# rahul-rwat/ESMStereo

Measured on AMD Instinct MI355X. Metric: stereo pairs/sec at 384×1248 maxdisp=192; EPE vs reference, higher is better.
Workload: dtype f32; 1 GPU; hot path: cost volume -> 3D stems -> 3D hourglass -> regression -> ESM upsampler (models/ESMStereo.py:700-745), ESMStereo-S gwc 384x1248 md192 B1; variant=S, cv=gwc, global_batch=1, height=384, width=1248, maxdisp=192, parallelism=dp1, graph=True

## Files before the change

### esmstereo_amd/csrc/conv_pair2.hip

```cpp
#include "conv_direct.h"

namespace esm {
namespace conv {
namespace {

constexpr int kP2Threads = 256;
constexpr int kHintPairReg = 1 << 29;

__device__ __forceinline__ float regress_px(const float* __restrict__ cp, int D, int sc) {
#pragma clang fp contract(off)
    float acc = 0.f;
    for (int d0 = 0; d0 < D; d0 += 16) {
        float v[16];
#pragma unroll
        for (int k = 0; k < 16; ++k) v[k] = d0 + k < D ? cp[(d0 + k) * sc] : 0.f;
#pragma unroll
        for (int k = 0; k < 16; ++k)
            if (d0 + k < D) acc = acc + v[k] * static_cast<float>(d0 + k);
    }
    return acc;
}

template <int KA, int SA, int KB, int TH>
struct P2Geo {
// ... 89 lines not shown
        const float v = (ok ? p : a.w)[ok ? c : 0];
        vep = ok ? v : ((k & 1) ? 0.f : 1.f);
    }
    if constexpr (REG) {
#pragma unroll
        for (int i = 0; i < PI; ++i) {
            const int e = i * kP2Threads + tid;
            const int q = e % IC, r = (e / IC) % IR, c = e / (IC * IR);
            const int yi = yi0 + r, xi = xi0 + q;
            vi[i] = 0.f;
            if (e < NIN && c == 0 && yi >= 0 && yi < a.Hi && xi >= 0 && xi < a.Wi) {
                const float v = regress_px(sp0 + yi * sh0 + xi, a.src[0].C, sc0);
                vi[i] = v;
                const bool own_y = (bk_.y == 0 || yi >= yb0) && (bk_.y == static_cast<int>(gridDim.y) - 1 || yi < yb0 + TH);
                const bool own_x = (bk_.x == 0 || xi >= xb0) && (bk_.x == static_cast<int>(gridDim.x) - 1 || xi < xb0 + VB);
                if (own_y && own_x) a.out[b * a.ob + yi * a.oh + xi] = v;
            }
        }
    }
    __builtin_amdgcn_sched_barrier(0);
#pragma unroll
    for (int i = 0; i < PI; ++i) {
        const int e = i * kP2Threads + tid;
        if (e < NIN) in[(e / (IC * IR)) * ICS + ((e / IC) % IR) * ICP + e % IC] = vi[i];
    }
#pragma unroll
    for (int i = 0; i < PWA; ++i) {
        const int e = i * kP2Threads + tid;
        if (e < NWA) wa[e] = vwa[i];
    }
#pragma unroll
    for (int i = 0; i < PWB; ++i) wb[i * kP2Threads + tid] = vwb[i];
    if (tid < 64) ep[tid] = vep;
    __syncthreads();

    for (int i = wave; i < NA; i += kP2Threads / 64) {
        floatx4 acc[2] = {floatx4{0.f, 0.f, 0.f, 0.f}, floatx4{0.f, 0.f, 0.f, 0.f}};
        const float* ib = in + kq * ICS + i * SA * ICP + n * SA;
        const float* wp = wa + kq * 16 + n;
        const int kca = (cin + 3) >> 2;
        if constexpr (TA > 1) {
            if (cin == 1) {
                const float* ib0 = in + i * SA * ICP + n * SA;
#pragma unroll
                for (int kc = 0; kc < (TA + 3) / 4; ++kc) {
                    const int t = 4 * kc + kq;
                    const bool tv = t < TA;
                    const int tt = tv ? t : 0;
                    const float bv = ib0[(tt / KA) * ICP + tt % KA];
                    const float av = wa[tt * CINMAX * 16 + n];
                    acc[kc & 1] = __builtin_amdgcn_mfma_f32_16x16x4f32(tv ? av : 0.f, tv ? bv : 0.f, acc[kc & 1], 0, 0, 0);
                }
            } else {
                for (int kc = 0; kc < kca; ++kc) {
#pragma unroll
                    for (int t = 0; t < TA; ++t) {
                        const int ky = t / KA, kx = t % KA;
                        const float bv = ib[4 * kc * ICS + ky * ICP + kx];
                        const float av = wp[(t * CINMAX + 4 * kc) * 16];
                        acc[t & 1] = __builtin_amdgcn_mfma_f32_16x16x4f32(av, bv, acc[t & 1], 0, 0, 0);
                    }
                }
            }
        } else {
            for (int kc = 0; kc < kca; kc += 2) {
                acc[0] = __builtin_amdgcn_mfma_f32_16x16x4f32(wp[4 * kc * 16], ib[4 * kc * ICS], acc[0], 0, 0, 0);
                if (kc + 1 < kca)
                    acc[1] = __builtin_amdgcn_mfma_f32_16x16x4f32(wp[4 * (kc + 1) * 16], ib[4 * (kc + 1) * ICS], acc[1],
                                                                  0, 0, 0);
            }
        }
        const int ya = ya0 + i, xa = xa0 + n;
        const bool inside = ya >= 0 && ya < a.Ho && xa >= 0 && xa < a.Wo;
#pragma unroll
        for (int j = 0; j < 4; ++j) {
            const int co = 4 * kq + j;
            const float v = act_t<ESM_ACT_GELU>((acc[0][j] + acc[1][j]) * ep[co] + ep[16 + co], 0);
            at[co * ACS + i * AR + n] = inside ? v : 0.f;
        }
    }
    __syncthreads();

    for (int t = wave; t < TH; t += kP2Threads / 64) {
        floatx4 acc[2] = {floatx4{0.f, 0.f, 0.f, 0.f}, floatx4{0.f, 0.f, 0.f, 0.f}};
        const float* ab = at + kq * ACS + t * AR + n;
        const float* wp = wb + kq * 16 + n;
#pragma unroll
        for (int kc = 0; kc < 4; ++kc)
#pragma unroll
            for (int tp = 0; tp < TB; ++tp) {
                const int dy = tp / KB, dx = tp % KB;
                const float bv = ab[4 * kc * ACS + dy * AR + dx];
                const float av = wp[(tp * 16 + 4 * kc) * 16];
                acc[tp & 1] = __builtin_amdgcn_mfma_f32_16x16x4f32(av, bv, acc[tp & 1], 0, 0, 0);
            }
        const int yb = yb0 + t, xb = xb0 + n;
        const bool ok = yb < bd.Ho && xb < bd.Wo && n < VB;
        const __amdgpu_buffer_rsrc_t ro = __builtin_amdgcn_make_buffer_rsrc(
            bd.out + b * bd.ob, static_cast<short>(0),
            4 * ((bd.Cout - 1) * static_cast<int>(bd.oc) + (bd.Ho - 1) * static_cast<int>(bd.oh) + bd.Wo), 0x00020000);
#pragma unroll
        for (int j = 0; j < 4; ++j) {
            const int co = 4 * kq + j;
            const float v = act_t<ESM_ACT_GELU>((acc[0][j] + acc[1][j]) * ep[32 + co] + ep[48 + co], 0);
            const unsigned o = (ok && co < bd.Cout) ? 4u * (co * static_cast<int>(bd.oc) + yb * static_cast<int>(bd.oh) + xb)
                                                    : kOOB;
            store_b32(__float_as_uint(v), ro, static_cast<int>(o), 0);
        }
    }
}

template <int KA, int SA, int KB, int TH, int CINMAX, bool REG = false>
int launch_p2(const esm_conv_desc& a, const esm_conv_desc& b, hipStream_t s) {
    using G = P2Geo<KA, SA, KB, TH>;
    const size_t lds = sizeof(float) * (static_cast<size_t>(CINMAX) * G::ICS + KA * KA * CINMAX * 16 + KB * KB * 256 +
                                        16 * G::ACS + 64);
    constexpr int VB = 16 - KB + 1;
    const dim3 grid(ceil_div(b.Wo, VB), ceil_div(b.Ho, TH), a.B);
    if (grid.y > 65535u || grid.z > 65535u) return arg_error("conv pair: grid too large");
    if constexpr (REG) {
        const int pr = b.ph + a.ph, pc = b.pw + a.pw;
        if (pr < 0 || pc < 0 || TH > G::IR - pr || VB > G::IC - pc ||
            (static_cast<int>(grid.y) - 1) * TH - pr + G::IR < a.Hi || (static_cast<int>(grid.x) - 1) * VB - pc + G::IC < a.Wi)
            return arg_error("conv pair: regressed map not covered by the tiles");
    }
    hipLaunchKernelGGL((pair2_kernel<KA, SA, KB, TH, CINMAX, REG>), grid, dim3(kP2Threads), lds, s, a, b);
    return check_launch("conv pair");
}

template <int KA, int SA, int KB>
int launch_p2_k(const esm_conv_desc& a, const esm_conv_desc& b, hipStream_t s) {
    const long long tiles4 = static_cast<long long>(ceil_div(b.Wo, 16 - KB + 1)) * ceil_div(b.Ho, 4) * a.B;
    const int thsel = (b.hint >> 26) & 3;
    const bool small = thsel ? thsel == 1 : tiles4 < 256;
    const bool tall = thsel == 3 && a.Cin <= 16;
    if constexpr (KA == 5 && KB == 3) {
        if (a.hint & kHintPairReg) {
            if (tall) return launch_p2<KA, SA, KB, 8, 4, true>(a, b, s);
            return small ? launch_p2<KA, SA, KB, 2, 4, true>(a, b, s) : launch_p2<KA, SA, KB, 4, 4, true>(a, b, s);
        }
    }
    if (tall) return a.Cin <= 4 ? launch_p2<KA, SA, KB, 8, 4>(a, b, s) : launch_p2<KA, SA, KB, 8, 16>(a, b, s);
    if (a.Cin <= 4) return small ? launch_p2<KA, SA, KB, 2, 4>(a, b, s) : launch_p2<KA, SA, KB, 4, 4>(a, b, s);
    if (a.Cin <= 16) return small ? launch_p2<KA, SA, KB, 2, 16>(a, b, s) : launch_p2<KA, SA, KB, 4, 16>(a, b, s);
    if (a.Cin <= 32) return small ? launch_p2<KA, SA, KB, 2, 32>(a, b, s) : launch_p2<KA, SA, KB, 4, 32>(a, b, s);
    if constexpr (KA == 1) {
        if (a.Cin > 48) return small ? launch_p2<KA, SA, KB, 2, 64>(a, b, s) : launch_p2<KA, SA, KB, 4, 64>(a, b, s);
    }
    return small ? launch_p2<KA, SA, KB, 2, 48>(a, b, s) : launch_p2<KA, SA, KB, 4, 48>(a, b, s);
}

}

bool pair2_ok(const esm_conv_desc& a, const esm_conv_desc& b) {
    const bool a3 = a.kd > 1 || a.Di > 1 || a.Do > 1, b3 = b.kd > 1 || b.Di > 1 || b.Do > 1;
    if (a3 || b3 || a.transposed || b.transposed || a.shuffle > 1 || b.shuffle > 1) return false;
    if (a.Cout != 16 || a.Cin < 1 || a.Cin > (a.kh == 1 ? 64 : 48) || b.Cin != 16 || b.Cout < 1 || b.Cout > 16)
        return false;
    if (!((a.kh == 3 && (a.stride == 1 || a.stride == 2)) || ((a.kh == 1 || a.kh == 5) && a.stride == 1))) return false;
    if (a.ph != a.pw || b.ph != b.pw || b.stride != 1 || (b.kh != 1 && b.kh != 3)) return false;
    if (a.act != ESM_ACT_GELU || b.act != ESM_ACT_GELU) return false;
    if (a.mul || a.res || a.up || a.out2 || a.post_scale != 1.f) return false;
    if (b.mul || b.res || b.up || b.out2 || b.post_scale != 1.f || !b.out) return false;
    if (b.Hi != a.Ho || b.Wi != a.Wo || b.B != a.B) return false;
    if (b.Ho != b.Hi + 2 * b.ph - b.kh + 1 || b.Wo != b.Wi + 2 * b.pw - b.kw + 1) return false;
    if (a.nsrc > 1)
        for (int i = 0; i < a.nsrc; ++i)
            if (a.src[i].C % 4) return false;
    if (a.hint & kHintPairReg) {
        if (a.kh != 5 || b.kh != 3 || a.Cin != 1 || a.nsrc != 1 || a.src[0].C < 1 || !a.out || a.out == b.out)
            return false;
        if (static_cast<long long>(a.src[0].C) * a.src[0].sc >= (1LL << 31) || a.src[0].sh >= (1 << 28)) return false;
    }
    const long long last = (b.Cout - 1) * b.oc + (b.Ho - 1) * b.oh + b.Wo;
    return 4 * last < static_cast<long long>(kOOB) && b.oc < (1 << 28) && b.oh < (1 << 28);
}

int launch_pair2(const esm_conv_desc& a, const esm_conv_desc& b, hipStream_t s) {
    if (!pair2_ok(a, b)) return arg_error("conv pair: unsupported pair");
    if (a.kh == 5) return b.kh == 3 ? launch_p2_k<5, 1, 3>(a, b, s) : launch_p2_k<5, 1, 1>(a, b, s);
    if (a.kh == 1) return b.kh == 3 ? launch_p2_k<1, 1, 3>(a, b, s) : launch_p2_k<1, 1, 1>(a, b, s);
    if (a.stride == 2) return b.kh == 3 ? launch_p2_k<3, 2, 3>(a, b, s) : launch_p2_k<3, 2, 1>(a, b, s);
    return b.kh == 3 ? launch_p2_k<3, 1, 3>(a, b, s) : launch_p2_k<3, 1, 1>(a, b, s);
}

}
}

extern "C" int esm_conv_pair2_f32(const esm_conv_desc* a, const esm_conv_desc* b, void* stream) {
    if (!a || !b) return esm::arg_error("conv pair: null descriptor");
    return esm::conv::launch_pair2(*a, *b, esm::as_stream(stream));
}
```

### esmstereo_amd/engine.py

```python
from __future__ import annotations

import contextlib
import ctypes
import json
import math
import os
import threading
from dataclasses import dataclass
from typing import Dict, List, Optional, Sequence, Tuple

import torch

from . import _lib
from ._lib import (ACT_GELU, ACT_NONE, ACT_RELU, ACT_RELU6, ACT_SIGMOID, ACT_SILU, EsmConfDesc, EsmConvDesc, EsmShuffleConvDesc,
                   EsmShuffleTailDesc, EsmSmixDesc, check, lib)

__all__ = ["Ctx", "PackedConv", "pack_conv", "run_conv", "run_smix", "run_fmnet", "run_shuffle_tail", "pack_shuffle_tail",
           "ACT_NONE", "ACT_GELU", "ACT_SILU", "ACT_RELU", "ACT_SIGMOID", "ACT_RELU6", "run_dwconv", "cached_pack", "run_convt_1x1",
           "convt_1x1_supported", "pack_conv_split", "run_conv_forked",
           "forked_packs", "run_side_partial"]


def _rup(x: int, m: int) -> int:
    return (x + m - 1) // m * m
# ... 479 lines not shown
        raise ValueError("conv: 1..3 sources")
    x0 = srcs[0]
    if x0.dim() != nd + 2:
        raise ValueError(f"conv: expected a {nd + 2}-D input, got shape {tuple(x0.shape)}")
    dev = x0.device
    B = int(x0.shape[0])
    Di, Hi, Wi = _spatial(x0, nd)
    cin = 0
    for i, s in enumerate(srcs):
        require_device(s, "conv input")
        if s.dim() != nd + 2 or int(s.shape[0]) != B or _spatial(s, nd) != (Di, Hi, Wi):
            raise RuntimeError(f"Sizes of tensors must match except in dimension 1 (conv sources "
                               f"{[tuple(t.shape) for t in srcs]})")
        st = s.stride()
        d.src[i].ptr = s.data_ptr()
        d.src[i].C = int(s.shape[1])
        d.src[i].sb, d.src[i].sc = st[0], st[1]
        d.src[i].sd = st[2] if nd == 3 else 0
        d.src[i].sh = st[-2]
        cin += int(s.shape[1])
    if cin != pc.cin:
        raise RuntimeError(f"conv: input has {cin} channels, layer expects {pc.cin}")
    require_on(dev, "conv", *srcs, pc.w, pc.scale, pc.shift, out, mul, res, up, out2, pre)
    d.nsrc = max(1, len(srcs))
    d.B, d.Cin = B, cin
    d.Di, d.Hi, d.Wi = Di, Hi, Wi
    k, s, p = pc.k, pc.stride, pc.pad
    if pc.transposed:
        if (k, s, p) != (4, 2, 1):
            raise ValueError("transposed conv: only k=4 s=2 p=1")
        Do, Ho, Wo = (2 * Di if nd == 3 else 1), 2 * Hi, 2 * Wi
    else:
        Ho, Wo = (Hi + 2 * p - k) // s + 1, (Wi + 2 * p - k) // s + 1
        Do = (Di + 2 * p - k) // s + 1 if nd == 3 else 1
    if min(Do, Ho, Wo) <= 0:
        raise RuntimeError(f"conv: empty output for input extent {(B, cin, Di, Hi, Wi)}")
    d.Do, d.Ho, d.Wo = Do, Ho, Wo
    d.kd = k if nd == 3 else 1
    d.kh = d.kw = k
    d.stride, d.transposed = s, int(pc.transposed)
    d.pd = p if nd == 3 else 0
    d.ph = d.pw = p
    d.Cout, d.cin_pad, d.cout_pad = pc.cout, pc.cin_pad, pc.cout_pad
    d.w = pc.w.data_ptr()
    d.scale = pc.scale.data_ptr() if pc.scale is not None else None
    d.shift = pc.shift.data_ptr() if pc.shift is not None else None
    d.act = pc.act
    r = int(shuffle)
    d.shuffle = r
    if out is None and alloc_out:
        if r > 1:
            if pc.cout % (r * r):
                raise ValueError("pixel shuffle: Cout not divisible by r^2")
            out = ctx.empty(B, pc.cout // (r * r), Ho * r, Wo * r)
        else:
            out = ctx.empty(B, pc.cout, Do, Ho, Wo) if nd == 3 else ctx.empty(B, pc.cout, Ho, Wo)
    if out is not None:
        require_device(out, "conv output")
        require_on(dev, "conv output", out)
        ost = out.stride()
        d.out = out.data_ptr()
        d.ob, d.oc = ost[0], ost[1]
        d.od = ost[2] if nd == 3 else 0
        d.oh = ost[-2]
    if mul is not None:
        require_device(mul, "conv mul")
        d.mul = mul.data_ptr()
        d.mb, d.mc, d.mh = mul.stride(0), mul.stride(1), mul.stride(-2)
    if res is not None:
        require_device(res, "conv residual")
        if out is None or tuple(res.shape) != tuple(out.shape):
            raise ValueError("conv: residual shape must match the output")
        rs = res.stride()
        d.res = res.data_ptr()
        d.rb, d.rc = rs[0], rs[1]
        d.rd = rs[2] if nd == 3 else 0
        d.rh = rs[-2]
    if up is not None:
        require_device(up, "conv bilinear source")
        d.up = up.data_ptr()
        d.up_h, d.up_w, d.up_f = int(up.shape[-2]), int(up.shape[-1]), int(up_f)
        d.ub, d.uh = up.stride(0), up.stride(-2)
        if d.up_h * up_f != Ho or d.up_w * up_f != Wo:
            raise ValueError("conv: bilinear source extent x factor must equal the output extent")
    d.post_scale = float(post_scale)
    if out2 is not None:
        require_device(out2, "conv out2")
        if out2.stride() != out.stride() or out2.shape != out.shape:
            raise ValueError("conv: out2 must have the output's shape and strides")
        d.out2 = out2.data_ptr()
        d.post_scale2 = float(post_scale2)
    if pre is not None:
        require_device(pre, "conv pre")
        if nd != 2 or pc.transposed or shuffle > 1 or up is not None or tuple(pre.shape) != (B, pc.cout, Ho, Wo):
            raise ValueError("conv: a partial sum (pre) is [B, Cout, Ho, Wo] of a 2-D, non-transposed conv")
        d.pre = pre.data_ptr()
        d.prb, d.prc, d.prh = pre.stride(0), pre.stride(1), pre.stride(2)
    key = conv_key(d, nd)
    d.hint = int(hint) if hint else HINT_SET.get(tag, TUNED_HINTS.get(key, 0))
    if (B * max(Di * Hi * Wi, Do * Ho * Wo) >= XCD_SLAB_MIN_PIX and (nd == 2 or XCD_SLAB_3D)) or \
            (nd == 3 and XCD_SLAB_3D and pc.cin >= 32 and B * Do * Ho * Wo >= XCD_SLAB_MIN_VOX_WIDE) or \
            tag in XCD_SLAB_OPS:
        d.hint |= HINT_XCD_SLAB
    ctx.hold(pc.w, pc.scale, pc.shift, *srcs, out, out2, mul, res, up, pre)
    taps = pc.k ** nd
    if pc.transposed:
        macs = B * Di * Hi * Wi * pc.cin * pc.cout * taps
    else:
        macs = B * Do * Ho * Wo * pc.cin * pc.cout * taps
    in_bytes = 4 * B * cin * Di * Hi * Wi
    out_bytes = 4 * B * pc.cout * Do * Ho * Wo * (2 if out2 is not None else 1)
    extra = 4 * sum(t.numel() for t in (res, mul, up, pre) if t is not None)
    w_bytes = 4 * pc.cin * pc.cout * taps
    meta = dict(name=tag, kind="conv", flops=2 * macs, bytes=in_bytes + out_bytes + extra + w_bytes,
                shape=f"{'T' if pc.transposed else ''}{nd}d k{pc.k}s{pc.stride} {cin}->{pc.cout} "
                      f"in {Di}x{Hi}x{Wi} out {Do}x{Ho}x{Wo}",
                reads=_spans(*srcs, mul, res, up, pre), writes=_spans(out, out2), key=key, hint=d.hint)
    return d, out, meta


GWC_STEM_ENABLED = _ab("ESM_GWC_STEM", "1") != "0"
GWC_STEM_WLDS = _ab("ESM_GWC_STEM_WLDS", "0") == "1"


def gwc_stem_supported(pc: PackedConv, L: torch.Tensor, G: int, D: int, att) -> bool:
    if att is not None or pc.nd != 3 or pc.transposed or (pc.k, pc.stride, pc.pad) != (3, 1, 1):
        return False
    B, C, H, W = (int(v) for v in L.shape)
    if pc.cin != G or G % 4 or C != 2 * G or pc.cout > 8 or not L.is_contiguous():
        return False
    return B * D * H * W >= (1 << 16) and 4 * C * H * W < (1 << 30) and 4 * pc.cout * D * H * W < (1 << 30)


def run_gwc_stem(ctx: Ctx, pc: PackedConv, L: torch.Tensor, R: torch.Tensor, G: int, D: int,
                 tag: str = "gwc_volume+group_stem", hint: int = 0) -> torch.Tensor:
    B, C, H, W = (int(v) for v in L.shape)
    if tuple(R.shape) != (B, C, H, W) or not R.is_contiguous() or not L.is_contiguous():
        raise ValueError("gwc_stem: L and R must be contiguous tensors of one shape")
    virt = L.as_strided((B, G, D, H, W), (0, 0, 0, 0, 1))
    d, out, meta = _conv_desc(ctx, pc, [virt], tag=tag, hint=hint)
    d.hint &= HINT_XCD_SLAB | (3 << 26) | ((1 << 28) if hint else 0)
    if GWC_STEM_WLDS:
        d.hint |= 1 << 28
    vol_flops = 2 * B * C * D * H * W
    meta.update(kind="gwc_stem", flops=meta["flops"] + vol_flops,
                bytes=4 * B * 2 * C * H * W + 4 * B * pc.cout * D * H * W + 4 * pc.cin * pc.cout * 27,
                reads=_spans(L, R), shape=f"gwc G{G} D{D} + " + meta["shape"])
    ctx.meta.append(meta)
    ctx.gwc_stem(d, L, R, C, G)
    return out


PAIR2_ENABLED = _ab("ESM_PAIR2", "1") != "0"


def pair2_supported(pa: PackedConv, pb: PackedConv, srcs: Sequence[torch.Tensor]) -> bool:
    if not PAIR2_ENABLED or pa.nd != 2 or pb.nd != 2 or pa.transposed or pb.transposed:
        return False
    if pa.cout != 16 or pb.cin != 16 or pb.cout > 16 or pa.cin > (64 if pa.k == 1 else 48):
        return False
    if not ((pa.k == 3 and pa.stride in (1, 2)) or (pa.k in (1, 5) and pa.stride == 1)):
        return False
    if pb.stride != 1 or pb.k not in (1, 3) or pa.act != ACT_GELU or pb.act != ACT_GELU:
        return False
    return len(srcs) == 1 or all(int(t.shape[1]) % 4 == 0 for t in srcs)


def pair2_auto(pa: PackedConv, pb: PackedConv, srcs: Sequence[torch.Tensor]) -> bool:
    if not pair2_supported(pa, pb, srcs):
        return False
    B = int(srcs[0].shape[0])
    Ho = (int(srcs[0].shape[2]) + 2 * pa.pad - pa.k) // pa.stride + 1
    Wo = (int(srcs[0].shape[3]) + 2 * pa.pad - pa.k) // pa.stride + 1
    light = pa.cin * pa.k * pa.k
    return pb.k == 1 or (light <= 25 and pa.stride == 1) or (pa.k == 1 and B * Ho * Wo <= 8192)


CONVT1X1_ENABLED = _ab("ESM_CONVT_1X1", "1") != "0"
CONVT1X1_PAIRED = _ab("ESM_CONVT_1X1_PAIRED", "1") == "1"
CONVT1X1_MAX_EXTRA = 48

FORK_ENABLED = _ab("ESM_FORK", "0") == "1"


def convt_1x1_supported(pa: PackedConv, pb: PackedConv, extra: Sequence[torch.Tensor]) -> bool:
    if not CONVT1X1_ENABLED or not pa.transposed or pb.transposed or (pa.k, pa.stride, pa.pad) != (4, 2, 1):
        return False
    wide = pa.cout > 16 or pb.cout > 16
    if pa.act != ACT_GELU or pa.scale is None or pa.shift is None or pa.cout > 32 or pa.cout % 4:
        return False
    if (pb.k, pb.stride, pb.pad) != (1, 1, 0) or pb.act != ACT_GELU or pb.cout > 32 or pb.nd != pa.nd:
        return False
    if wide and (pa.nd != 3 or pa.cout < 2):
        return False
    cx = sum(int(t.shape[1]) for t in extra)
    return 1 <= len(extra) <= 2 and all(int(t.shape[1]) % 4 == 0 for t in extra) and \
        4 <= cx <= (32 if wide else CONVT1X1_MAX_EXTRA)


def run_convt_1x1(ctx: Ctx, pa: PackedConv, srcs: Sequence[torch.Tensor], pb: PackedConv, extra: Sequence[torch.Tensor],
                  tags: Tuple[str, str] = ("convT", "conv1x1"), pre: Optional[torch.Tensor] = None) -> torch.Tensor:
    da, _, ma = _conv_desc(ctx, pa, srcs, tag=tags[0], alloc_out=False)
    nd = pa.nd
    e0 = extra[0]
    geo = (int(e0.shape[0]), pa.cout) + tuple(int(v) for v in e0.shape[2:])
    virt = srcs[0].as_strided(geo, (0,) * (len(geo) - 1) + (1,))
    db, out, mb = _conv_desc(ctx, pb, [virt, *extra], tag=tags[1], pre=pre)
    db.hint = 0
    B = int(e0.shape[0])
    vox = math.prod(int(v) for v in e0.shape[2:])
    full = 4 * B * pa.cout * int(da.Ho) * int(da.Wo) * (int(da.Do) if nd == 3 else 1)
    name = f"{tags[0]}+{'.'.join(tags[1].split('.')[-2:])}"
    ctx.meta.append(dict(name=name, kind="conv_up1", flops=ma["flops"] + mb["flops"],
                         bytes=ma["bytes"] - full + mb["bytes"] - 4 * B * pa.cout * vox,
                         shape=f"{ma['shape']} + {mb['shape']}", reads=ma["reads"] + _spans(*extra), writes=mb["writes"],
                         key=ma["key"] + " | " + mb["key"], hint=da.hint))
    if ctx._submit():
        if ctx.plan:
            ctx._placed(check(lib.esm_plan_add_convt_1x1(ctx.plan, ctypes.byref(da), ctypes.byref(db)), "plan_add_convt_1x1"))
        else:
            check(lib.esm_convt_1x1_f32(ctypes.byref(da), ctypes.byref(db), ctx.stream), "convt_1x1")
    return out


def forked_packs(owner: torch.nn.Module, conv: torch.nn.Module, bn: Optional[torch.nn.Module], act: int, cm: int,
                 cs: int) -> Tuple[PackedConv, PackedConv]:
    def build():
        return (pack_conv_split(conv, None, act, cm, cm + cs), pack_conv_split(conv, bn, act, 0, cm))
    return cached_pack(owner, f"fork{cm}", [conv, bn], build)


def run_side_partial(ctx: Ctx, p_side: PackedConv, side: torch.Tensor, tag: str, cm: int) -> torch.Tensor:
    with ctx.side():
        part = run_conv(ctx, p_side, [side], tag=tag + "[side]")
    ctx.meta[-1].update(layer=tag, split=(cm, cm + p_side.cin))
    ctx.join_next()
    return part


def run_conv_forked(ctx: Ctx, owner: torch.nn.Module, conv: torch.nn.Module, bn: Optional[torch.nn.Module], act: int,
                    main: Sequence[torch.Tensor], side: torch.Tensor, tag: str = "conv") -> torch.Tensor:
    cm = sum(int(t.shape[1]) for t in main)
    p_side, p_main = forked_packs(owner, conv, bn, act, cm, int(side.shape[1]))
    part = run_side_partial(ctx, p_side, side, tag, cm)
    out = run_conv(ctx, p_main, list(main), pre=part, tag=tag)
    ctx.meta[-1].update(layer=tag, split=(0, cm))
    return out


PAIR_REGRESS_ENABLED = _ab("ESM_PAIR_REGRESS", "1") != "0"
PAIR2_TH = {sel: tuple(x for x in _ab(f"ESM_PAIR2_TH{n}", "").split(",") if x)
            for sel, n in ((1, 2), (2, 4), (3, 8))}
HINT_PAIR_REGRESS = 1 << 29


def run_pair2(ctx: Ctx, pa: PackedConv, srcs: Sequence[torch.Tensor], pb: PackedConv,
              tags: Tuple[str, str] = ("convA", "convB"), force: bool = False,
              regress: Optional[torch.Tensor] = None) -> torch.Tensor:
    take = pair2_supported(pa, pb, srcs) if force else pair2_auto(pa, pb, srcs)
    if regress is not None:
        B_, D_, H_, W_ = (int(v) for v in regress.shape)
        init = srcs[0]
        fuse = (take and PAIR_REGRESS_ENABLED and len(srcs) == 1 and pa.k == 5 and pb.k == 3 and pa.cin == 1
                and regress.stride(3) == 1 and tuple(init.shape) == (B_, 1, H_, W_) and init.stride(3) == 1)
        if not fuse:
            ctx.regression(0, regress, init, B_, D_, H_, W_)
            regress = None
    if not take:
        return run_conv(ctx, pb, [run_conv(ctx, pa, srcs, tag=tags[0])], tag=tags[1])
    da, _, ma = _conv_desc(ctx, pa, srcs, tag=tags[0], alloc_out=False)
    da.hint &= ~HINT_PAIR_REGRESS
    B = int(srcs[0].shape[0])
    geo = (B, pa.cout) + ((int(da.Do),) if pa.nd == 3 else ()) + (int(da.Ho), int(da.Wo))
    virt = srcs[0].as_strided(geo, (0,) * (len(geo) - 1) + (1,))
    db, out, mb = _conv_desc(ctx, pb, [virt], tag=tags[1])
    db.hint &= ~(3 << 26)
    for sel, subs in PAIR2_TH.items():
        if any(x in tags[0] for x in subs):
            db.hint |= sel << 26
    mid = 4 * B * pa.cout * int(da.Ho) * int(da.Wo) * (int(da.Do) if pa.nd == 3 else 1)
    name = f"{tags[0]}+{tags[1].rsplit('.', 1)[-1]}"
    flops, byts, reads, writes = ma["flops"] + mb["flops"], ma["bytes"] - mid + mb["bytes"] - mid, ma["reads"], mb["writes"]
    if regress is not None:
        require_on(init.device, "pair regression", regress)
        st = regress.stride()
        da.src[0].ptr, da.src[0].C = regress.data_ptr(), D_
        da.src[0].sb, da.src[0].sc, da.src[0].sh = st[0], st[1], st[2]
        da.out = init.data_ptr()
        da.ob, da.oc, da.oh = init.stride(0), init.stride(1), init.stride(2)
        da.hint |= HINT_PAIR_REGRESS
        ctx.hold(regress, init)
        name = "disparity_regression+" + name
        flops += 2 * B_ * D_ * H_ * W_
        byts += 4 * B_ * D_ * H_ * W_
        reads, writes = _spans(regress), writes + _spans(init)
    ctx.meta.append(dict(name=name, kind="conv_pair", flops=flops, bytes=byts, shape=f"pair {ma['shape']} + {mb['shape']}",
                         reads=reads, writes=writes, key=ma["key"] + " | " + mb["key"], hint=0))
    ctx.pair2(da, db)
    return out


def run_dwconv(ctx: Ctx, x: torch.Tensor, w: torch.Tensor, scale: Optional[torch.Tensor], shift: Optional[torch.Tensor],
               k: int, stride: int, pad: int, act: int, tag: str = "dwconv") -> torch.Tensor:
    if stride <= 0 or k <= 0 or not 0 <= pad < k:
        raise ValueError("dwconv: stride and K must be positive, 0 <= pad < K")
    if x.dim() != 4 or x.stride(3) != 1:
        raise ValueError("dwconv: a [B, C, H, W] input with unit W stride")
    require_device(x, "dwconv input")
    B, C, H, W = (int(v) for v in x.shape)
    Ho, Wo = (H + 2 * pad - k) // stride + 1, (W + 2 * pad - k) // stride + 1
    out = ctx.empty(B, C, Ho, Wo)
    require_on(x.device, "dwconv", x, w, scale, shift, out)
    d = _lib.EsmDwconvDesc()
    d.x, d.xb, d.xc, d.xh = x.data_ptr(), x.stride(0), x.stride(1), x.stride(2)
    d.w = w.data_ptr()
    d.scale = scale.data_ptr() if scale is not None else None
    d.shift = shift.data_ptr() if shift is not None else None
    d.out, d.ob, d.oc, d.oh = out.data_ptr(), out.stride(0), out.stride(1), out.stride(2)
    d.B, d.C, d.H, d.W, d.K, d.stride, d.pad, d.act, d.Ho, d.Wo = B, C, H, W, k, stride, pad, act, Ho, Wo
    ctx.meta.append(dict(name=tag, kind="dwconv", flops=2 * B * C * Ho * Wo * k * k,
                         bytes=4 * (x.numel() + out.numel() + C * k * k), reads=_spans(x), writes=_spans(out)))
    ctx.dwconv(d)
    return out


@dataclass
class SmixStage:
    ln_w: torch.Tensor
    fc0_w: torch.Tensor
    fc0_b: torch.Tensor
    fc2_w: torch.Tensor
    fc2_b: torch.Tensor


def run_smix(ctx: Ctx, x: torch.Tensor, stages: Sequence[SmixStage], *, dw: Optional[Tuple[torch.Tensor, torch.Tensor]] = None,
             res: Optional[torch.Tensor] = None, out: Optional[torch.Tensor] = None, tag: str = "smix") -> torch.Tensor:
    require_device(x, "smix input")
    if not x.is_contiguous():
        raise ValueError("smix: input must be contiguous")
    B, C, H, W = (int(v) for v in x.shape)
    if out is None:
        out = ctx.empty(B, C, H, W)
    d = EsmSmixDesc()
    d.x, d.out = x.data_ptr(), out.data_ptr()
    if res is not None:
        require_device(res, "smix residual")
        if not res.is_contiguous() or res.shape != x.shape:
            raise ValueError("smix: residual must be contiguous and shaped like the input")
        d.res = res.data_ptr()
    if dw is not None:
        d.dw_w, d.dw_b = dw[0].data_ptr(), dw[1].data_ptr()
        d.dw_k = int(dw[0].shape[-1])
    if len(stages) > _lib.SMIX_MAX_STAGES:
        raise ValueError("smix: at most 2 stages per launch")
    require_on(x.device, "smix", x, out, res, *(dw or ()),
               *[t for st in stages for t in (st.ln_w, st.fc0_w, st.fc0_b, st.fc2_w, st.fc2_b)])
    d.nstages = len(stages)
    for i, st in enumerate(stages):
        d.stage[i].ln_w = st.ln_w.data_ptr()
        d.stage[i].fc0_w, d.stage[i].fc0_b = st.fc0_w.data_ptr(), st.fc0_b.data_ptr()
        d.stage[i].fc2_w, d.stage[i].fc2_b = st.fc2_w.data_ptr(), st.fc2_b.data_ptr()
        ctx.hold(st.ln_w, st.fc0_w, st.fc0_b, st.fc2_w, st.fc2_b)
    d.B, d.C, d.H, d.W = B, C, H, W
    ctx.hold(x, out, res, *(dw or ()))
    npix = B * H * W
    ctx.meta.append(dict(name=tag, kind="smix", flops=npix * (2 * C * C * len(stages) + (2 * C * d.dw_k ** 2 if dw else 0)),
                         bytes=4 * npix * C * (3 if res is not None else 2), shape=f"C{C} {H}x{W} dw{d.dw_k}",
                         reads=_spans(x, res), writes=_spans(out)))
    ctx.smix(d)
    return out


FM2_MIN_PIX = int(_ab("ESM_FM2_MIN_PIX", "16384"))


def run_fmnet(ctx: Ctx, x: torch.Tensor, stages: Sequence[SmixStage], dw0: Tuple[torch.Tensor, torch.Tensor],
              dw1: Tuple[torch.Tensor, torch.Tensor], out: Optional[torch.Tensor] = None,
              tag: str = "fmnet", conv: Optional[Tuple[torch.Tensor, ...]] = None,
              two_launch: Optional[bool] = None) -> torch.Tensor:
    require_device(x, "fmnet input")
    if not x.is_contiguous():
        raise ValueError("fmnet: input must be contiguous")
    if len(stages) != 4:
        raise ValueError("fmnet: four mlp stages")
    B, C, H, W = (int(v) for v in x.shape)
    if out is None:
        out = ctx.empty(B, C, H, W)
    d = _lib.EsmFmnetDesc()
    d.x, d.out = x.data_ptr(), out.data_ptr()
    d.dw_w[0], d.dw_b[0] = dw0[0].data_ptr(), dw0[1].data_ptr()
    d.dw_w[1], d.dw_b[1] = dw1[0].data_ptr(), dw1[1].data_ptr()
    d.dw_k = int(dw0[0].shape[-1])
    if int(dw1[0].shape[-1]) != d.dw_k:
        raise ValueError("fmnet: both SMLayers need the same depthwise kernel")
    require_on(x.device, "fmnet", x, out, *dw0, *dw1,
               *[t for st in stages for t in (st.ln_w, st.fc0_w, st.fc0_b, st.fc2_w, st.fc2_b)])
    for i, st in enumerate(stages):
        d.stage[i].ln_w = st.ln_w.data_ptr()
        d.stage[i].fc0_w, d.stage[i].fc0_b = st.fc0_w.data_ptr(), st.fc0_b.data_ptr()
        d.stage[i].fc2_w, d.stage[i].fc2_b = st.fc2_w.data_ptr(), st.fc2_b.data_ptr()
        ctx.hold(st.ln_w, st.fc0_w, st.fc0_b, st.fc2_w, st.fc2_b)
    d.B, d.C, d.H, d.W = B, C, H, W
    if conv is not None:
        w0, b0, w2, b2 = conv
        hid = int(w0.shape[0])
        if tuple(w0.shape) != (hid, C, 3, 3) or tuple(w2.shape[:2]) != (C, hid) or hid != C + 16:
            raise ValueError("fmnet: FMBlock.conv must be Conv2d(C, C+16, 3) and Conv2d(C+16, C, 1)")
        for t in conv:
            if not t.is_contiguous():
                raise ValueError("fmnet: conv weights must be contiguous")
        require_on(x.device, "fmnet conv", *conv)
        d.conv0_w, d.conv0_b, d.conv2_w, d.conv2_b = (t.data_ptr() for t in conv)
        d.hid = hid
        ctx.hold(*conv)
        if two_launch is None:
            two_launch = B * H * W >= FM2_MIN_PIX
        if two_launch:
            work = ctx.empty(B, C, H, W)
            d.work = work.data_ptr()
            ctx.hold(work)
    ctx.hold(x, out, *dw0, *dw1)
    npix = B * H * W
    flops = 2 * C * C * 4 + 2 * 2 * C * d.dw_k ** 2 + (2 * d.hid * C * 9 + 2 * C * d.hid if conv is not None else 0)
    ctx.meta.append(dict(name=tag, kind="fmnet", flops=npix * flops,
                         bytes=4 * npix * C * 2 + 4 * (sum(int(t.numel()) for t in conv) if conv is not None else 0),
                         shape=f"C{C} {H}x{W} dw{d.dw_k} x2" + (f" +conv{d.hid}" if conv is not None else ""),
                         reads=_spans(x), writes=_spans(out), launches=2 if d.work else 1))
    ctx.fmnet(d)
    return out
# ... 167 lines not shown
```

Before: 3250 pairs/s.

## Add K-split MFMA fused conv pair kernel for small 3x3 conv pairs

```diff
diff --git a/esmstereo_amd/csrc/conv_pair2.hip b/esmstereo_amd/csrc/conv_pair2.hip
--- a/esmstereo_amd/csrc/conv_pair2.hip
+++ b/esmstereo_amd/csrc/conv_pair2.hip
@@ -265,7 +265,7 @@
 
 }
 
-bool pair2_ok(const esm_conv_desc& a, const esm_conv_desc& b) {
+bool pair2_lds_ok(const esm_conv_desc& a, const esm_conv_desc& b) {
     const bool a3 = a.kd > 1 || a.Di > 1 || a.Do > 1, b3 = b.kd > 1 || b.Di > 1 || b.Do > 1;
     if (a3 || b3 || a.transposed || b.transposed || a.shuffle > 1 || b.shuffle > 1) return false;
     if (a.Cout != 16 || a.Cin < 1 || a.Cin > (a.kh == 1 ? 64 : 48) || b.Cin != 16 || b.Cout < 1 || b.Cout > 16)
@@ -289,8 +289,21 @@
     return 4 * last < static_cast<long long>(kOOB) && b.oc < (1 << 28) && b.oh < (1 << 28);
 }
 
+bool pairk_ok(const esm_conv_desc& a, const esm_conv_desc& b);
+int launch_pairk(const esm_conv_desc& a, const esm_conv_desc& b, hipStream_t s);
+
+constexpr int kHintPairK = 1 << 28;
+
+bool pair2_ok(const esm_conv_desc& a, const esm_conv_desc& b) {
+    if (a.pre || b.pre) return false;
+    return pair2_lds_ok(a, b) || pairk_ok(a, b);
+}
+
 int launch_pair2(const esm_conv_desc& a, const esm_conv_desc& b, hipStream_t s) {
-    if (!pair2_ok(a, b)) return arg_error("conv pair: unsupported pair");
+    if (a.pre || b.pre) return arg_error("conv pair: a partial sum (pre) is not supported on either conv");
+    const bool lds = pair2_lds_ok(a, b);
+    if (((b.hint & kHintPairK) || !lds) && !(a.hint & kHintPairReg) && pairk_ok(a, b)) return launch_pairk(a, b, s);
+    if (!lds) return arg_error("conv pair: unsupported pair");
     if (a.kh == 5) return b.kh == 3 ? launch_p2_k<5, 1, 3>(a, b, s) : launch_p2_k<5, 1, 1>(a, b, s);
     if (a.kh == 1) return b.kh == 3 ? launch_p2_k<1, 1, 3>(a, b, s) : launch_p2_k<1, 1, 1>(a, b, s);
     if (a.stride == 2) return b.kh == 3 ? launch_p2_k<3, 2, 3>(a, b, s) : launch_p2_k<3, 2, 1>(a, b, s);
diff --git a/esmstereo_amd/csrc/conv_pairk.hip b/esmstereo_amd/csrc/conv_pairk.hip
--- /dev/null
+++ b/esmstereo_amd/csrc/conv_pairk.hip
@@ -0,0 +1,313 @@
+#include <algorithm>
+
+#include "conv_direct.h"
+
+namespace esm {
+namespace conv {
+namespace {
+
+constexpr int kPkAR = 18;
+constexpr int kPkVB = 14;
+constexpr size_t kPkMaxLds = 64 * 1024;
+constexpr int kPkWaves = 16;
+
+__device__ __forceinline__ int pk_div(int n, unsigned m) {
+    return m ? static_cast<int>(__umulhi(static_cast<unsigned>(n), m)) : n;
+}
+
+inline unsigned pk_magic(int d) {
+    return d <= 1 ? 0u : static_cast<unsigned>(((1ull << 32) + static_cast<unsigned long long>(d) - 1) / d);
+}
+
+inline int pk_acs(int np, int na) {
+    const int s = np * na * kPkAR;
+    return s + ((16 - s % 32) + 32) % 32;
+}
+
+struct PkGeo {
+    int th;
+    int acs;
+    int red;
+    unsigned m_ga, m_gb, m_do;
+    unsigned m_ca, m_cb;
+};
+
+template <int MT>
+__device__ __forceinline__ void pk_load_wb(float (&av)[9][MT], __amdgpu_buffer_rsrc_t wrs, unsigned wl, int wtap,
+                                           int cout_pad, int g, int dz) {
+#pragma unroll
+    for (int t = 0; t < 9; ++t)
+#pragma unroll
+        for (int mt = 0; mt < MT; ++mt)
+            av[t][mt] = buf_load_s(wrs, wl, 4 * ((dz * 9 + t) * wtap + 4 * g * cout_pad + 16 * mt));
+}
+
+template <bool D3, int SA, int MT, int NW>
+__global__ void __launch_bounds__(64 * NW) pairk_kernel(const esm_conv_desc a, const esm_conv_desc bd, const PkGeo geo) {
+    constexpr int NP = D3 ? 3 : 1;
+    constexpr int KDT = D3 ? 3 : 1;
+    constexpr int TAPS = KDT * 9;
+    extern __shared__ __attribute__((aligned(16))) float lds[];
+    float* red = lds;
+    float* at = red + geo.red;
+    const int TH = geo.th, NA = TH + 2, ACS = geo.acs;
+    const int GA = (a.Cin + 3) >> 2, GB = (bd.Cin + 3) >> 2;
+    const int CPA = 4 * ((a.Cout + 3) >> 2), CPB = 4 * ((bd.Cout + 3) >> 2);
+    float* ep = at + CPA * ACS;
+
+    const int tid = static_cast<int>(threadIdx.x);
+    const int lane = tid & 63, wave = __builtin_amdgcn_readfirstlane(tid >> 6);
+    const int n16 = lane & 15, kq = lane >> 4;
+    const Blk3 bk_ = xcd_block((a.hint & kHintXcd) != 0);
+    const int xb0 = bk_.x * kPkVB, yb0 = bk_.y * TH;
+    const int b = pk_div(bk_.z, geo.m_do);
+    const int zb = bk_.z - b * bd.Do;
+
+    if (tid < 128) {
+        const int k = tid >> 5, c = tid & 31;
+        const float* p = k == 0 ? a.scale : (k == 1 ? a.shift : (k == 2 ? bd.scale : bd.shift));
+        const int cn = k < 2 ? a.Cout : bd.Cout;
+        const bool ok = p != nullptr && c < cn;
+        const float v = (ok ? p : a.w)[ok ? c : 0];
+        ep[tid] = ok ? v : ((k & 1) ? 0.f : 1.f);
+    }
+
+    const int plo = D3 ? max(0, 1 - zb) : 0, phi = D3 ? min(3, a.Do + 1 - zb) : 1;
+    const int ilo = max(0, 1 - yb0), ihi = min(NA, a.Ho + 1 - yb0);
+    const int nvr = ihi - ilo;
+    const int ntask = (phi - plo) * nvr * GA;
+
+    const int xa = xb0 - 1 + n16;
+    unsigned xoff[3];
+#pragma unroll
+    for (int t = 0; t < 3; ++t) {
+        const int xi = xa * SA - a.pw + t;
+        xoff[t] = (xa >= 0 && xa < a.Wo && xi >= 0 && xi < a.Wi) ? 4u * xi : kOOB;
+    }
+    const int wtap = a.cin_pad * a.cout_pad;
+    const __amdgpu_buffer_rsrc_t wrs =
+        __builtin_amdgcn_make_buffer_rsrc(const_cast<float*>(a.w), static_cast<short>(0), 4 * TAPS * wtap, 0x00020000);
+    const unsigned wl = 4u * (kq * a.cout_pad + n16);
+    const int ns = a.nsrc;
+    const int lo1 = a.src[0].C, lo2 = lo1 + (ns > 1 ? a.src[1].C : 0);
+
+    for (int t = wave; t < ntask; t += NW) {
+        const int seg = pk_div(t, geo.m_ga);
+        const int g = t - seg * GA;
+        const int pp = (seg >= nvr ? 1 : 0) + (seg >= 2 * nvr ? 1 : 0);
+        const int za = zb - 1 + plo + pp, ya = yb0 - 1 + ilo + (seg - pp * nvr);
+        const int c0 = 4 * g;
+        const int s = (ns > 1 && c0 >= lo1) ? ((ns > 2 && c0 >= lo2) ? 2 : 1) : 0;
+        const int lo = s == 0 ? 0 : (s == 1 ? lo1 : lo2);
+        const float* sp = s == 0 ? a.src[0].ptr : (s == 1 ? a.src[1].ptr : a.src[2].ptr);
+        const int sC = s == 0 ? a.src[0].C : (s == 1 ? a.src[1].C : a.src[2].C);
+        const long long sb = s == 0 ? a.src[0].sb : (s == 1 ? a.src[1].sb : a.src[2].sb);
+        const int sc = static_cast<int>(s == 0 ? a.src[0].sc : (s == 1 ? a.src[1].sc : a.src[2].sc));
+        const int sd = static_cast<int>(s == 0 ? a.src[0].sd : (s == 1 ? a.src[1].sd : a.src[2].sd));
+        const int sh = static_cast<int>(s == 0 ? a.src[0].sh : (s == 1 ? a.src[1].sh : a.src[2].sh));
+        const int span = 4 * ((sC - 1) * sc + (D3 ? (a.Di - 1) * sd : 0) + (a.Hi - 1) * sh + a.Wi);
+        const __amdgpu_buffer_rsrc_t rs =
+            __builtin_amdgcn_make_buffer_rsrc(const_cast<float*>(sp + b * sb), static_cast<short>(0), span, 0x00020000);
+        const int cl = c0 - lo + kq;
+        const unsigned chv = (c0 + kq < a.Cin && cl < sC) ? 4u * cl * sc : kOOB;
+
+        float bv[TAPS], av[TAPS][MT];
+#pragma unroll
+        for (int dz = 0; dz < KDT; ++dz) {
+            const int zi = D3 ? za * SA - a.pd + dz : 0;
+            const bool zok = !D3 || (zi >= 0 && zi < a.Di);
+#pragma unroll
+            for (int dy = 0; dy < 3; ++dy) {
+                const int yi = ya * SA - a.ph + dy;
+                const int roff = (zok && yi >= 0 && yi < a.Hi) ? 4 * ((D3 ? zi * sd : 0) + yi * sh) : static_cast<int>(kOOB);
+#pragma unroll
+                for (int dx = 0; dx < 3; ++dx) {
+                    const int tap = (dz * 3 + dy) * 3 + dx;
+                    bv[tap] = buf_load_s(rs, chv + xoff[dx], roff);
+#pragma unroll
+                    for (int mt = 0; mt < MT; ++mt)
+                        av[tap][mt] = buf_load_s(wrs, wl, 4 * (tap * wtap + c0 * a.cout_pad + 16 * mt));
+                }
+            }
+        }
+        __builtin_amdgcn_sched_barrier(0);
+        floatx4 acc[2][MT];
+#pragma unroll
+        for (int c = 0; c < 2; ++c)
+#pragma unroll
+            for (int mt = 0; mt < MT; ++mt) acc[c][mt] = floatx4{0.f, 0.f, 0.f, 0.f};
+#pragma unroll
+        for (int tap = 0; tap < TAPS; ++tap)
+#pragma unroll
+            for (int mt = 0; mt < MT; ++mt)
+                acc[tap & 1][mt] = __builtin_amdgcn_mfma_f32_16x16x4f32(av[tap][mt], bv[tap], acc[tap & 1][mt], 0, 0, 0);
+        float* rp = red + t * CPA * 16 + n16;
+#pragma unroll
+        for (int mt = 0; mt < MT; ++mt)
+#pragma unroll
+            for (int j = 0; j < 4; ++j) {
+                const int co = 16 * mt + 4 * kq + j;
+                if (co < CPA) rp[co * 16] = acc[0][mt][j] + acc[1][mt][j];
+            }
+    }
+
+    const int NPB = D3 ? 3 : 1;
+    const int ntb = TH * GB * NPB;
+    const int wtapb = bd.cin_pad * bd.cout_pad;
+    const __amdgpu_buffer_rsrc_t wrsb =
+        __builtin_amdgcn_make_buffer_rsrc(const_cast<float*>(bd.w), static_cast<short>(0), 4 * TAPS * wtapb, 0x00020000);
+    const unsigned wlb = 4u * (kq * bd.cout_pad + n16);
+    float avb[9][MT];
+    {
+        const int tg = pk_div(wave, D3 ? 0x55555556u : 0u);
+        const int dz = wave - tg * NPB;
+        const int g = tg - pk_div(tg, geo.m_gb) * GB;
+        if (wave < ntb) pk_load_wb<MT>(avb, wrsb, wlb, wtapb, bd.cout_pad, g, dz);
+    }
+    __syncthreads();
+
+    {
+        const int nel = NP * NA * CPA * 16;
+        for (int e = tid; e < nel; e += 64 * NW) {
+            const int sgi = pk_div(e, geo.m_ca);
+            const int r = e - sgi * CPA * 16;
+            const int co = r >> 4, n = r & 15;
+            const int p = D3 ? (sgi >= NA ? 1 : 0) + (sgi >= 2 * NA ? 1 : 0) : 0;
+            const int i = sgi - p * NA;
+            const int xc = xb0 - 1 + n;
+            const bool ok = p >= plo && p < phi && i >= ilo && i < ihi && xc >= 0 && xc < a.Wo && co < a.Cout;
+            float v = 0.f;
+            if (ok) {
+                const float* rp = red + ((p - plo) * nvr + (i - ilo)) * GA * CPA * 16 + r;
+                v = rp[0];
+                for (int g = 1; g < GA; ++g) v = v + rp[g * CPA * 16];
+                v = gelu_erf(v * ep[co] + ep[32 + co]);
+            }
+            at[co * ACS + sgi * kPkAR + n] = v;
+        }
+    }
+    __syncthreads();
+
+    for (int tb = wave; tb < ntb; tb += NW) {
+        const int tg = pk_div(tb, D3 ? 0x55555556u : 0u);
+        const int dz = tb - tg * NPB;
+        const int tr = pk_div(tg, geo.m_gb);
+        const int g = tg - tr * GB;
+        if (tb != wave) pk_load_wb<MT>(avb, wrsb, wlb, wtapb, bd.cout_pad, g, dz);
+        const float* ab = at + (4 * g + kq) * ACS + (dz * NA + tr) * kPkAR + n16;
+        float bvb[9];
+#pragma unroll
+        for (int t = 0; t < 9; ++t) bvb[t] = ab[(t / 3) * kPkAR + t % 3];
+        __builtin_amdgcn_sched_barrier(0);
+        floatx4 acc[2][MT];
+#pragma unroll
+        for (int c = 0; c < 2; ++c)
+#pragma unroll
+            for (int mt = 0; mt < MT; ++mt) acc[c][mt] = floatx4{0.f, 0.f, 0.f, 0.f};
+#pragma unroll
+        for (int t = 0; t < 9; ++t)
+#pragma unroll
+            for (int mt = 0; mt < MT; ++mt)
+                acc[t & 1][mt] = __builtin_amdgcn_mfma_f32_16x16x4f32(avb[t][mt], bvb[t], acc[t & 1][mt], 0, 0, 0);
+        float* rp = red + tb * CPB * 16 + n16;
+#pragma unroll
+        for (int mt = 0; mt < MT; ++mt)
+#pragma unroll
+            for (int j = 0; j < 4; ++j) {
+                const int co = 16 * mt + 4 * kq + j;
+                if (co < CPB) rp[co * 16] = acc[0][mt][j] + acc[1][mt][j];
+            }
+    }
+    __syncthreads();
+
+    {
+        const __amdgpu_buffer_rsrc_t ro = __builtin_amdgcn_make_buffer_rsrc(
+            bd.out + b * bd.ob, static_cast<short>(0),
+            4 * ((bd.Cout - 1) * static_cast<int>(bd.oc) + (D3 ? (bd.Do - 1) * static_cast<int>(bd.od) : 0) +
+                 (bd.Ho - 1) * static_cast<int>(bd.oh) + bd.Wo),
+            0x00020000);
+        const int nel = TH * CPB * 16;
+        const int per = GB * NPB;
+        for (int e = tid; e < nel; e += 64 * NW) {
+            const int tr = pk_div(e, geo.m_cb);
+            const int r = e - tr * CPB * 16;
+            const int co = r >> 4, n = r & 15;
+            const float* rp = red + tr * per * CPB * 16 + r;
+            float v = rp[0];
+            for (int k = 1; k < per; ++k) v = v + rp[k * CPB * 16];
+            v = gelu_erf(v * ep[64 + co] + ep[96 + co]);
+            const int yb = yb0 + tr, xb = xb0 + n;
+            const bool ok = n < kPkVB && xb < bd.Wo && yb < bd.Ho && co < bd.Cout;
+            const unsigned vo = ok ? 4u * (co * static_cast<int>(bd.oc) + xb) : kOOB;
+            const int so = 4 * ((D3 ? zb * static_cast<int>(bd.od) : 0) + min(yb, bd.Ho - 1) * static_cast<int>(bd.oh));
+            store_b32(__float_as_uint(v), ro, static_cast<int>(vo), so);
+        }
+    }
+}
+
+size_t pk_geo(const esm_conv_desc& a, const esm_conv_desc& b, bool d3, int th, PkGeo* geo) {
+    const int np = d3 ? 3 : 1, na = th + 2;
+    const int ga = (a.Cin + 3) / 4, gb = (b.Cin + 3) / 4;
+    const int cpa = 4 * ((a.Cout + 3) / 4), cpb = 4 * ((b.Cout + 3) / 4);
+    const int segs = std::min(np, a.Do) * std::min(na, a.Ho);
+    const int red = std::max(segs * ga * cpa * 16, th * gb * np * cpb * 16);
+    const int acs = pk_acs(np, na);
+    if (geo) *geo = PkGeo{th, acs, red, pk_magic(ga), pk_magic(gb), pk_magic(b.Do), pk_magic(cpa * 16), pk_magic(cpb * 16)};
+    return sizeof(float) * (static_cast<size_t>(red) + static_cast<size_t>(cpa) * acs + 128);
+}
+
+template <bool D3, int SA, int MT>
+int launch_pk(const esm_conv_desc& a, const esm_conv_desc& b, hipStream_t s) {
+    const int tiles_w = ceil_div(b.Wo, kPkVB);
+    const long long planes = static_cast<long long>(b.Do) * a.B;
+    const int sel = (b.hint >> 26) & 3;
+    int th = sel == 3 ? 4 : sel;
+    if (!th) {
+        th = 1;
+        while (th < 4 && tiles_w * static_cast<long long>(ceil_div(b.Ho, th)) * planes > 256) th *= 2;
+    }
+    while (th > 1 && pk_geo(a, b, D3, th, nullptr) > kPkMaxLds) th /= 2;
+    PkGeo geo;
+    const size_t lds = pk_geo(a, b, D3, th, &geo);
+    if (lds > kPkMaxLds) return arg_error("conv pair (K-split): tile does not fit LDS");
+    const dim3 grid(tiles_w, ceil_div(b.Ho, th), static_cast<unsigned>(planes));
+    if (grid.y > 65535u || planes > 65535) return arg_error("conv pair (K-split): grid too large");
+    hipLaunchKernelGGL((pairk_kernel<D3, SA, MT, kPkWaves>), grid, dim3(64 * kPkWaves), lds, s, a, b, geo);
+    return check_launch("conv pair (K-split)");
+}
+
+}
+
+bool pairk_ok(const esm_conv_desc& a, const esm_conv_desc& b) {
+    const bool a3 = a.kd > 1 || a.Di > 1 || a.Do > 1, b3 = b.kd > 1 || b.Di > 1 || b.Do > 1;
+    if (a3 != b3 || a.transposed || b.transposed || a.shuffle > 1 || b.shuffle > 1) return false;
+    if (a.kh != 3 || a.kw != 3 || b.kh != 3 || b.kw != 3 || a.kd != (a3 ? 3 : 1) || b.kd != (a3 ? 3 : 1)) return false;
+    if ((a.stride != 1 && a.stride != 2) || b.stride != 1) return false;
+    if (a.ph != 1 || a.pw != 1 || b.ph != 1 || b.pw != 1 || (a3 && (a.pd != 1 || b.pd != 1))) return false;
+    if (a.Cin < 1 || a.Cin > 48 || a.Cout < 1 || a.Cout > 32 || b.Cin != a.Cout || b.Cout < 1 || b.Cout > 32) return false;
+    if (a.act != ESM_ACT_GELU || b.act != ESM_ACT_GELU) return false;
+    if (a.mul || a.res || a.up || a.out2 || a.post_scale != 1.f || a.pre) return false;
+    if (b.mul || b.res || b.up || b.out2 || b.post_scale != 1.f || b.pre || !b.out) return false;
+    if (a.nsrc < 1 || a.nsrc > ESM_MAX_SRC || !direct_ok(a)) return false;
+    int cs = 0;
+    for (int i = 0; i < a.nsrc; ++i) cs += a.src[i].C;
+    if (cs < a.Cin) return false;
+    if (b.B != a.B || b.Di != a.Do || b.Hi != a.Ho || b.Wi != a.Wo || b.Do != b.Di || b.Ho != b.Hi || b.Wo != b.Wi) return false;
+    if (a.Do < 1 || a.Ho < 1 || a.Wo < 1 || a.B < 1) return false;
+    const long long last = (b.Cout - 1) * b.oc + (a3 ? (b.Do - 1) * b.od : 0) + (b.Ho - 1) * b.oh + b.Wo;
+    if (4 * last >= static_cast<long long>(kOOB) || b.oc >= (1 << 28) || b.od >= (1 << 28) || b.oh >= (1 << 28)) return false;
+    return pk_geo(a, b, a3, 1, nullptr) <= kPkMaxLds;
+}
+
+int launch_pairk(const esm_conv_desc& a, const esm_conv_desc& b, hipStream_t s) {
+    if (!pairk_ok(a, b)) return arg_error("conv pair (K-split): unsupported pair");
+    const bool d3 = a.kd > 1;
+    const bool mt2 = a.Cout > 16 || b.Cout > 16;
+#define ESM_PK(D, S) (mt2 ? launch_pk<D, S, 2>(a, b, s) : launch_pk<D, S, 1>(a, b, s))
+    if (d3) return a.stride == 2 ? ESM_PK(true, 2) : ESM_PK(true, 1);
+    return a.stride == 2 ? ESM_PK(false, 2) : ESM_PK(false, 1);
+#undef ESM_PK
+}
+
+}
+}
diff --git a/esmstereo_amd/engine.py b/esmstereo_amd/engine.py
--- a/esmstereo_amd/engine.py
+++ b/esmstereo_amd/engine.py
@@ -655,22 +655,66 @@
 
 
 PAIR2_ENABLED = _ab("ESM_PAIR2", "1") != "0"
+PAIRK_ENABLED = _ab("ESM_PAIRK", "1") != "0"
+PAIRK_MAX_VOX = int(_ab("ESM_PAIRK_MAX_VOX", "4096"))
+HINT_PAIRK = 1 << 28
+
+
+def _pair_out(pa: PackedConv, srcs: Sequence[torch.Tensor]) -> Tuple[int, ...]:
+    ext = tuple((int(v) + 2 * pa.pad - pa.k) // pa.stride + 1 for v in srcs[0].shape[2:])
+    return ((1,) + ext) if pa.nd == 2 else ext
+
+
+def _pair2_lds_supported(pa: PackedConv, pb: PackedConv, srcs: Sequence[torch.Tensor]) -> bool:
+    if pa.nd != 2 or pb.nd != 2 or pa.transposed or pb.transposed:
+        return False
+    if pa.cout != 16 or pb.cin != 16 or pb.cout > 16 or pa.cin > (64 if pa.k == 1 else 48):
+        return False
+    if not ((pa.k == 3 and pa.stride in (1, 2)) or (pa.k in (1, 5) and pa.stride == 1)):
+        return False
+    if pb.stride != 1 or pb.k not in (1, 3) or pa.act != ACT_GELU or pb.act != ACT_GELU:
+        return False
+    return len(srcs) == 1 or all(int(t.shape[1]) % 4 == 0 for t in srcs)
+
+
+def pairk_supported(pa: PackedConv, pb: PackedConv, srcs: Sequence[torch.Tensor]) -> bool:
+    if not PAIR2_ENABLED or pa.nd != pb.nd or pa.transposed or pb.transposed:
+        return False
+    if (pa.k, pa.pad) != (3, 1) or (pb.k, pb.pad, pb.stride) != (3, 1, 1) or pa.stride not in (1, 2):
+        return False
+    if not (1 <= pa.cin <= 48 and 1 <= pa.cout <= 32 and pb.cin == pa.cout and 1 <= pb.cout <= 32):
+        return False
+    if pa.act != ACT_GELU or pb.act != ACT_GELU:
+        return False
+    if len(srcs) > 1 and any(int(t.shape[1]) % 4 for t in srcs):
+        return False
+    Do, Ho, _ = _pair_out(pa, srcs)
+    if min(_pair_out(pa, srcs)) < 1:
+        return False
+    np_ = 3 if pa.nd == 3 else 1
+    ga, gb = (pa.cin + 3) // 4, (pb.cin + 3) // 4
+    cpa, cpb = 4 * ((pa.cout + 3) // 4), 4 * ((pb.cout + 3) // 4)
+    red = max(min(np_, Do) * min(3, Ho) * ga * cpa * 16, gb * np_ * cpb * 16)
+    acs = np_ * 3 * 18
+    acs += (16 - acs % 32) % 32
+    return 4 * (red + cpa * acs + 128) <= 64 * 1024
 
 
 def pair2_supported(pa: PackedConv, pb: PackedConv, srcs: Sequence[torch.Tensor]) -> bool:
-    if not PAIR2_ENABLED or pa.nd != 2 or pb.nd != 2 or pa.transposed or pb.transposed:
-        return False
-    if pa.cout != 16 or pb.cin != 16 or pb.cout > 16 or pa.cin > (64 if pa.k == 1 else 48):
-        return False
-    if not ((pa.k == 3 and pa.stride in (1, 2)) or (pa.k in (1, 5) and pa.stride == 1)):
-        return False
-    if pb.stride != 1 or pb.k not in (1, 3) or pa.act != ACT_GELU or pb.act != ACT_GELU:
-        return False
-    return len(srcs) == 1 or all(int(t.shape[1]) % 4 == 0 for t in srcs)
+    return PAIR2_ENABLED and (_pair2_lds_supported(pa, pb, srcs) or pairk_supported(pa, pb, srcs))
+
+
+def pairk_auto(pa: PackedConv, pb: PackedConv, srcs: Sequence[torch.Tensor]) -> bool:
+    if not PAIRK_ENABLED or pa.nd != 2 or not pairk_supported(pa, pb, srcs):
+        return False
+    vox = int(srcs[0].shape[0]) * math.prod(_pair_out(pa, srcs))
+    return vox <= PAIRK_MAX_VOX
 
 
 def pair2_auto(pa: PackedConv, pb: PackedConv, srcs: Sequence[torch.Tensor]) -> bool:
-    if not pair2_supported(pa, pb, srcs):
+    if pairk_auto(pa, pb, srcs):
+        return True
+    if not PAIR2_ENABLED or not _pair2_lds_supported(pa, pb, srcs):
         return False
     B = int(srcs[0].shape[0])
     Ho = (int(srcs[0].shape[2]) + 2 * pa.pad - pa.k) // pa.stride + 1
@@ -759,8 +803,13 @@
 
 def run_pair2(ctx: Ctx, pa: PackedConv, srcs: Sequence[torch.Tensor], pb: PackedConv,
               tags: Tuple[str, str] = ("convA", "convB"), force: bool = False,
-              regress: Optional[torch.Tensor] = None) -> torch.Tensor:
+              regress: Optional[torch.Tensor] = None, ksplit: Optional[bool] = None) -> torch.Tensor:
     take = pair2_supported(pa, pb, srcs) if force else pair2_auto(pa, pb, srcs)
+    if ksplit is None:
+        ksplit = take and regress is None and ((not force and pairk_auto(pa, pb, srcs)) or
+                                               not _pair2_lds_supported(pa, pb, srcs))
+    elif take and not (pairk_supported if ksplit else _pair2_lds_supported)(pa, pb, srcs):
+        raise ValueError("conv pair: the requested form does not run this pair")
     if regress is not None:
         B_, D_, H_, W_ = (int(v) for v in regress.shape)
         init = srcs[0]
@@ -777,7 +826,9 @@
     geo = (B, pa.cout) + ((int(da.Do),) if pa.nd == 3 else ()) + (int(da.Ho), int(da.Wo))
     virt = srcs[0].as_strided(geo, (0,) * (len(geo) - 1) + (1,))
     db, out, mb = _conv_desc(ctx, pb, [virt], tag=tags[1])
-    db.hint &= ~(3 << 26)
+    db.hint &= ~((3 << 26) | HINT_PAIRK)
+    if ksplit:
+        db.hint |= HINT_PAIRK
     for sel, subs in PAIR2_TH.items():
         if any(x in tags[0] for x in subs):
             db.hint |= sel << 26
```

Result: faster. 3292 pairs/s, median of 6 (+1.3%).
